# IBM/AdaMML

Measured on AMD Instinct MI355X. Metric: clips/sec (train fwd+bwd) RGB+Audio AdaMML @224^2, 5 seg, higher is better.
Workload: dtype bf16

## Files before the change

adamml_amd/csrc/conv_stem.hip:

```cpp
#include "common.h"
#include "../../include/adamml_hip.h"


namespace {

constexpr int NT = 256;
constexpr int KSTEPS = 7;
constexpr int KTOT = KSTEPS * 32;
constexpr int WROW = KTOT * 2 + 16;
constexpr int MAXPX = 256;
constexpr int SROW = 128 + 8;
constexpr int MAXSLOT = 6;

struct StemP {
    const bf16_t* x;
    const bf16_t* w;
    bf16_t* y;
    double* stats;
    int N, H, W, xc, OH, OW;
    int R;
    int tiles_per_img, total_tiles, tpb;
    int PW, PR;
    size_t gx, gy;
};

__global__ __launch_bounds__(NT, 2) void conv_stem_kernel(StemP p) {
    extern __shared__ __attribute__((aligned(16))) char smem[];
    char* s_w = smem;
    float* cs = reinterpret_cast<float*>(smem + 64 * WROW);
    char* s_patch = smem + 64 * WROW + 512;
    const int tid = threadIdx.x, lane = tid & 63, wave = tid >> 6;
    const int li = lane & 15, lg = lane >> 4;
    const int g = blockIdx.y;
    p.x += (size_t)g * p.gx;
    p.y += (size_t)g * p.gy;

    {
        constexpr int WSL = 64 * (KTOT / 8) / NT;
        static_assert(64 * (KTOT / 8) % NT == 0, "weight slots must divide evenly");
        bf16x8 wv[WSL];
#pragma unroll
        for (int l = 0; l < WSL; ++l) wv[l] = *reinterpret_cast<const bf16x8*>(p.w + (size_t)(tid + l * NT) * 8);
#pragma unroll
        for (int l = 0; l < WSL; ++l) {
            const int e = tid + l * NT;
            const int co = e / (KTOT / 8), ch = e - co * (KTOT / 8);
            *reinterpret_cast<bf16x8*>(s_w + co * WROW + ch * 16) = wv[l];
        }
    }
    if (tid < 128) cs[tid] = 0.f;

    const int pairs_per_row = p.PW >> 1;
    const int nslots = p.PR * pairs_per_row;
    int s_off[MAXSLOT], s_ih[MAXSLOT], s_iw[MAXSLOT];
#pragma unroll
    for (int l = 0; l < MAXSLOT; ++l) {
        const int e = tid + l * NT;
        const int pr = e / pairs_per_row, pc = (e - pr * pairs_per_row) * 2;
        s_ih[l] = e < nslots ? pr : -(1 << 20);
        s_iw[l] = pc - 3;
        s_off[l] = (pr * p.PW + pc) * 8;
    }
    s16x4 ra[MAXSLOT], rb[MAXSLOT];
    unsigned vmask = 0;
    auto load_patch = [&](int tile) {
        const int n = tile / p.tiles_per_img, tr = tile - n * p.tiles_per_img;
        const int ih0 = 2 * tr * p.R - 3;
        vmask = 0;
        const bf16_t* img = p.x + (size_t)n * p.H * p.W * p.xc;
#pragma unroll
        for (int l = 0; l < MAXSLOT; ++l) {
            const int ih = ih0 + s_ih[l], iw = s_iw[l];
            const bool rok = (unsigned)ih < (unsigned)p.H;
            const bf16_t* row = img + (size_t)min(max(ih, 0), p.H - 1) * p.W * p.xc;
            ra[l] = *reinterpret_cast<const s16x4*>(row + min(max(iw, 0), p.W - 1) * p.xc);
            rb[l] = *reinterpret_cast<const s16x4*>(row + min(max(iw + 1, 0), p.W - 1) * p.xc);
            vmask |= ((rok && (unsigned)iw < (unsigned)p.W) ? 1u : 0u) << (2 * l);
            vmask |= ((rok && (unsigned)(iw + 1) < (unsigned)p.W) ? 2u : 0u) << (2 * l);
        }
    };
    const int tile0 = blockIdx.x * p.tpb;
    if (tile0 < p.total_tiles) load_patch(tile0);
    int pixoff[4];
#pragma unroll
    for (int pt = 0; pt < 4; ++pt) {
        int q = (wave * 4 + pt) * 16 + li;
        if (q >= p.R * p.OW) q = 0;
        const int r = q / p.OW, c = q - r * p.OW;
        pixoff[pt] = ((2 * r) * p.PW + 2 * c + 2 * lg) * 8;
    }

    for (int it = 0; it < p.tpb; ++it) {
        const int tile = tile0 + it;
        if (tile >= p.total_tiles) break;
        const int n = tile / p.tiles_per_img, tr = tile - n * p.tiles_per_img;
        const int oh0 = tr * p.R;
        const int rows = min(p.R, p.OH - oh0);
        const int npx = rows * p.OW;
#pragma unroll
        for (int l = 0; l < MAXSLOT; ++l) {
            if (tid + l * NT < nslots) {
                union { struct { s16x4 a, b; } s; bf16x8 v; } u;
                u.s.a = (vmask >> (2 * l)) & 1u ? ra[l] : s16x4{0, 0, 0, 0};
                u.s.b = (vmask >> (2 * l)) & 2u ? rb[l] : s16x4{0, 0, 0, 0};
                *reinterpret_cast<bf16x8*>(s_patch + s_off[l]) = u.v;
            }
        }
        __syncthreads();
        if (it + 1 < p.tpb && tile + 1 < p.total_tiles) load_patch(tile + 1);

        f32x4 acc[4][4];
#pragma unroll
        for (int pt = 0; pt < 4; ++pt)
#pragma unroll
            for (int ct = 0; ct < 4; ++ct) acc[ct][pt] = f32x4{0.f, 0.f, 0.f, 0.f};
        const int rowbytes = p.PW * 8;
#pragma unroll
        for (int kh = 0; kh < KSTEPS; ++kh) {
            bf16x8 fw[4];
#pragma unroll
            for (int ct = 0; ct < 4; ++ct) fw[ct] = *reinterpret_cast<const bf16x8*>(s_w + (ct * 16 + li) * WROW + kh * 64 + lg * 16);
            bf16x8 fa[4];
#pragma unroll
            for (int pt = 0; pt < 4; ++pt) fa[pt] = *reinterpret_cast<const bf16x8*>(s_patch + pixoff[pt] + kh * rowbytes);
#pragma unroll
            for (int pt = 0; pt < 4; ++pt)
#pragma unroll
                for (int ct = 0; ct < 4; ++ct)
                    acc[ct][pt] = __builtin_amdgcn_mfma_f32_16x16x32_bf16(fw[ct], fa[pt], acc[ct][pt], 0, 0, 0);
        }
        __syncthreads();

#pragma unroll
        for (int pt = 0; pt < 4; ++pt) {
            const int q = (wave * 4 + pt) * 16 + li;
#pragma unroll
            for (int ct = 0; ct < 4; ++ct) {
                bf16x4 v = f32_to_bf4(acc[ct][pt]);
                if (q >= npx) v = bf16x4{0, 0, 0, 0};
                *reinterpret_cast<bf16x4*>(s_patch + q * SROW + (ct * 16 + lg * 4) * 2) = v;
            }
        }
        __syncthreads();
        bf16_t* ybase = p.y + ((size_t)n * p.OH + oh0) * p.OW * 64;
        for (int e = tid; e < npx * 8; e += NT) {
            const int q = e >> 3, ch = e & 7;
            const s16x4 lo = *reinterpret_cast<const s16x4*>(s_patch + q * SROW + ch * 16);
            const s16x4 hi = *reinterpret_cast<const s16x4*>(s_patch + q * SROW + ch * 16 + 8);
            union { struct { s16x4 a, b; } s; bf16x8 v; } u;
            u.s.a = lo; u.s.b = hi;
            *reinterpret_cast<bf16x8*>(ybase + (size_t)q * 64 + ch * 8) = u.v;
        }
        if (p.stats) {
            union { s16x4 h[2]; bf16x8 v; } ones;
            ones.h[0] = s16x4{0x3F80, 0x3F80, 0x3F80, 0x3F80};
            ones.h[1] = ones.h[0];
            const int trow = 8 * lg + (li >> 2);
            f32x4 dsum = {0.f, 0.f, 0.f, 0.f}, dsq = {0.f, 0.f, 0.f, 0.f};
            const int nps = (npx + 31) >> 5;
            for (int ps = 0; ps < nps; ++ps) {
                const char* fp = s_patch + (ps * 32 + trow) * SROW + (wave * 16 + 4 * (li & 3)) * 2;
                union { s16x4 h[2]; bf16x8 v; } f;
                f.h[0] = __builtin_amdgcn_ds_read_tr16_b64_v4i16((__attribute__((address_space(3))) s16x4*)(fp));
                f.h[1] = __builtin_amdgcn_ds_read_tr16_b64_v4i16((__attribute__((address_space(3))) s16x4*)(fp + 4 * SROW));
                dsum = __builtin_amdgcn_mfma_f32_16x16x32_bf16(ones.v, f.v, dsum, 0, 0, 0);
                dsq = __builtin_amdgcn_mfma_f32_16x16x32_bf16(f.v, f.v, dsq, 0, 0, 0);
            }
            if (lg == 0) cs[wave * 16 + li] += dsum[0];
            if ((li >> 2) == lg) {
                const int r = li & 3;
                cs[64 + wave * 16 + li] += r == 0 ? dsq[0] : r == 1 ? dsq[1] : r == 2 ? dsq[2] : dsq[3];
            }
        }
        __syncthreads();
    }
    if (p.stats) {
        __syncthreads();
        if (tid < 128) det_add(p.stats + (size_t)g * ADAMML_STAT_SLOTS * 128 + tid, 128, cs[tid]);
    }
}

struct StemWP {
    const bf16_t* x;
    const bf16_t* dz;
    float* ws;
    int N, H, W, xc, OH, OW, R, tiles_per_img, total_tiles, tpb, PW, PR;
};

constexpr int DZROW = 128 + 8;
constexpr int MAXDZ = 8;

__global__ __launch_bounds__(NT, 2) void conv_stem_wgrad_kernel(StemWP p) {
    extern __shared__ __attribute__((aligned(16))) char smem[];
    char* s_patch = smem;
    char* s_dz = smem + ((p.PR * p.PW * 8 + 15) & ~15);
    const int tid = threadIdx.x, lane = tid & 63, wave = tid >> 6;
    const int li = lane & 15, lg = lane >> 4;
    const int pairs_per_row = p.PW >> 1;
    const int nslots = p.PR * pairs_per_row;
    int s_off[MAXSLOT], s_ih[MAXSLOT], s_iw[MAXSLOT];
#pragma unroll
    for (int l = 0; l < MAXSLOT; ++l) {
        const int e = tid + l * NT;
        const int pr = e / pairs_per_row, pc = (e - pr * pairs_per_row) * 2;
        s_ih[l] = e < nslots ? pr : -(1 << 20);
        s_iw[l] = pc - 3;
        s_off[l] = (pr * p.PW + pc) * 8;
    }
    s16x4 ra[MAXSLOT], rb[MAXSLOT];
    bf16x8 rz[MAXDZ];
    unsigned vmask = 0;
    auto load_tile = [&](int tile) {
        const int n = tile / p.tiles_per_img, tr = tile - n * p.tiles_per_img;
// ... 128 lines not shown
    }
}

__global__ void pack_stem_weight_kernel(const float* w, bf16_t* out, int cin_true) {
    const int e = blockIdx.x * blockDim.x + threadIdx.x;
    if (e >= 64 * KTOT) return;
    const int c = e & 3, kw = (e >> 2) & 7, kh = (e >> 5) % 7, co = e / KTOT;
    float v = 0.f;
    if (kw < 7 && c < cin_true) v = w[((size_t)(co * cin_true + c) * 7 + kh) * 7 + kw];
    reinterpret_cast<__bf16*>(out)[e] = (__bf16)v;
}

}

extern "C" int adamml_pack_stem_weight(const float* w, void* out, int cout, int cin_true, hipStream_t stream) {
    if (!w || !out) return adamml_set_error(ADAMML_EINVAL, "pack_stem_weight: null argument");
    if (cout != 64 || cin_true < 1 || cin_true > 4)
        return adamml_set_error(ADAMML_EUNSUPPORTED, "pack_stem_weight: needs cout == 64 and 1..4 input channels (cout=%d cin=%d)", cout, cin_true);
    hipLaunchKernelGGL(pack_stem_weight_kernel, dim3(ceil_div(64 * KTOT, 256)), dim3(256), 0, stream, w, (bf16_t*)out, cin_true);
    return adamml_check_launch("pack_stem_weight");
}

extern "C" int adamml_conv_stem_supported(const adamml_conv_desc_t* d) {
    if (!d) return 0;
    if (d->KH != 7 || d->KW != 7 || d->stride != 2 || d->pad != 3 || d->Cout != 64 || (d->Cin != 8 && d->Cin != 4)) return 0;
    if (d->W % 2 || d->OW != d->W / 2 || d->OH != (d->H + 6 - 7) / 2 + 1 || d->OW > MAXPX || d->OW < 1) return 0;
    const int R = MAXPX / d->OW;
    const int PR = 2 * R + 5, PW = d->W + 6;
    const size_t patch = (size_t)PR * PW * 8, stage = (size_t)MAXPX * SROW;
    if (PR * (PW / 2) > MAXSLOT * NT) return 0;
    return 64 * WROW + 512 + (patch > stage ? patch : stage) <= 64 * 1024;
}

extern "C" int adamml_conv_stem_fwd(const adamml_conv_desc_t* d, const void* x, const void* w_stem_packed, void* y, double* stats,
                                    hipStream_t stream) {
    if (!d || !x || !w_stem_packed || !y) return adamml_set_error(ADAMML_EINVAL, "conv_stem_fwd: null argument");
    if (!adamml_conv_stem_supported(d))
        return adamml_set_error(ADAMML_EUNSUPPORTED, "conv_stem_fwd: needs a 7x7/2 pad 3 conv of a <=4-channel (8-padded) image to 64 "
                                "channels with even W <= %d*2 (H=%d W=%d Cin=%d Cout=%d)", MAXPX, d->H, d->W, d->Cin, d->Cout);
    StemP p;
    p.x = (const bf16_t*)x; p.w = (const bf16_t*)w_stem_packed; p.y = (bf16_t*)y; p.stats = stats;
    p.N = d->N; p.H = d->H; p.W = d->W; p.xc = d->Cin; p.OH = d->OH; p.OW = d->OW;
    p.R = MAXPX / d->OW;
    if (p.R > d->OH) p.R = d->OH;
    p.PR = 2 * p.R + 5; p.PW = d->W + 6;
    p.tiles_per_img = ceil_div(d->OH, p.R);
    p.total_tiles = d->N * p.tiles_per_img;
    if (p.total_tiles <= 0) return ADAMML_OK;
    const int groups = d->groups < 1 ? 1 : d->groups;
    p.gx = (size_t)d->N * d->H * d->W * d->Cin;
    p.gy = (size_t)d->N * d->OH * d->OW * 64;
    p.tpb = (int)(((long)p.total_tiles * groups + 1535) / 1536);
    if (p.tpb < 1) p.tpb = 1;
    const size_t patch = (size_t)p.PR * p.PW * 8, stage = (size_t)MAXPX * SROW;
    const size_t lds = 64 * WROW + 512 + (patch > stage ? patch : stage);
    hipLaunchKernelGGL(conv_stem_kernel, dim3(ceil_div(p.total_tiles, p.tpb), groups), dim3(NT), lds, stream, p);
    return adamml_check_launch("conv_stem_fwd");
}

static int stem_wgrad_blocks(const adamml_conv_desc_t* d, int* tpb_out) {
    const int R = MAXPX / d->OW > d->OH ? d->OH : MAXPX / d->OW;
    const long total = (long)(d->groups < 1 ? 1 : d->groups) * d->N * ceil_div(d->OH, R);
    int tpb = (int)((total + 767) / 768);
    if (tpb < 1) tpb = 1;
    *tpb_out = tpb;
    return (int)((total + tpb - 1) / tpb);
}

extern "C" size_t adamml_conv_stem_bwd_weight_workspace(const adamml_conv_desc_t* d) {
    if (!d || !adamml_conv_stem_supported(d)) return 0;
    int tpb;
    return (size_t)stem_wgrad_blocks(d, &tpb) * 64 * KTOT * sizeof(float);
}

extern "C" int adamml_conv_stem_bwd_weight(const adamml_conv_desc_t* d, const void* dz, const void* x, float* dw, int cin_true,
                                           void* workspace, size_t workspace_bytes, hipStream_t stream) {
    if (!d || !dz || !x || !dw || !workspace) return adamml_set_error(ADAMML_EINVAL, "conv_stem_bwd_weight: null argument");
    if (!adamml_conv_stem_supported(d) || cin_true < 1 || cin_true > 4)
        return adamml_set_error(ADAMML_EUNSUPPORTED, "conv_stem_bwd_weight: not a stem shape (see adamml_conv_stem_supported)");
    StemWP p;
    p.x = (const bf16_t*)x; p.dz = (const bf16_t*)dz; p.ws = (float*)workspace;
    p.N = d->N * (d->groups < 1 ? 1 : d->groups);
    p.H = d->H; p.W = d->W; p.xc = d->Cin; p.OH = d->OH; p.OW = d->OW;
    p.R = MAXPX / d->OW;
    if (p.R > d->OH) p.R = d->OH;
    p.PR = 2 * p.R + 5; p.PW = d->W + 6;
    p.tiles_per_img = ceil_div(d->OH, p.R);
    p.total_tiles = p.N * p.tiles_per_img;
    if (p.total_tiles <= 0) return ADAMML_OK;
    const int nblk = stem_wgrad_blocks(d, &p.tpb);
// ... 12 lines not shown
```

adamml_amd/hip.py:

```python
import ctypes
import os
from ctypes import c_void_p, c_int, c_int32, c_int64, c_float, c_double, c_size_t, c_char_p, POINTER, Structure, byref

import torch

_HERE = os.path.dirname(os.path.abspath(__file__))
LIB_PATH = os.environ.get("ADAMML_HIP_LIB") or os.path.join(_HERE, "libadamml_hip.so")

ACT_NONE, ACT_RELU, ACT_RELU6 = 0, 1, 2
STAT_SLOTS = 32


class ConvDesc(Structure):
    _fields_ = [(n, c_int32) for n in ("N", "H", "W", "Cin", "OH", "OW", "Cout", "KH", "KW", "stride", "pad", "up", "act",
                                      "accumulate", "groups", "in_gstride")]

    def __init__(self, *args, **kw):
        super().__init__(*args, **kw)
        if self.groups < 1:
            self.groups = 1


_P, _I, _F, _D, _Z, _L = c_void_p, c_int, c_float, c_double, c_size_t, c_int64
_DESC = POINTER(ConvDesc)

SIGNATURES = {
    "adamml_conv_fwd": [_DESC, _P, _P, _P, _P, _P, _P, _P],
    "adamml_conv_bwd_data": [_DESC, _P, _P, _P, _I, _P],
    "adamml_conv_fwd_bn_add": [_DESC, _P, _P, _P, _P, _P, _P, _P, _P, _I, _I, _P, _P, _P],
    "adamml_conv_fwd_bn_add_next": [_DESC, _P, _P, _P, _P, _P, _P, _P, _P, _I, _I, _P, _P, _P, _P, _P, _P],
    "adamml_conv_fwd_bn_add_tpool": [_DESC, _P, _P, _P, _P, _P, _P, _P, _P, _I, _I, _I, _P, _P, _P],
    "adamml_temporal_pool_bwd_code": [_P, _P, _P, _P, _I, _I, _I, _I, _I, _P],
    "adamml_temporal_pool_bwd_code_prod": [_P, _P, _P, _P, _P, _P, _P, _I, _I, _P, _P, _Z, _I, _I, _I, _I, _I, _I, _P],
    "adamml_copy2d": [_P, _Z, _P, _Z, _Z, _Z, _P],
    "adamml_gram_stats": [_P, _P, _P, _P, _I, _I, _I, _P],
    "adamml_gram_colsum": [_P, _P, _P, _I, _I, _P, _P, _Z, _I, _I, _P, _Z, _P],
    "adamml_conv_bwd_data_bn": [_DESC, _P, _P, _P, _P, _P, _I, _P, _P],
    "adamml_bn_bwd_affine": [_P, _P, _P, _I, _I, _P],
    "adamml_conv_bwd_data_dual": [_DESC, _P, _P, _P, _P, _P, _P, _I, _P, _P, _I, _P, _P],
    "adamml_conv_bwd_weight_grouped": [_DESC, _P, _P, _P, _I, _I, _P, _P, _P, _P, _I, _P, _Z, _P],
    "adamml_lazy_colsum": [_P, _P, _P, _I, _I, _P, _Z, _I, _I, _P],
    "adamml_alg_sumfix": [_P, _P, _P, _P, _I, _I, _I, _P],
    "adamml_alg_pack": [_P, _P, _P, _P, _P, _I, _I, _I, _P],
    "adamml_alg_wgrad_combine": [_P, _P, _P, _P, _P, _P, _P, _I, _I, _I, _P],
    "adamml_conv_bwd_data_alg": [_DESC, _P, _P, _P, _P, _P, _P, _P, _I, _P, _P, _I, _P, _P],
    "adamml_conv_bwd_data_res": [_DESC, _P, _P, _P, _I, _P, _P, _I, _P, _P, _P, _P, _P, _P, _P],
    "adamml_conv_bwd_data_res_prod": [_DESC, _P, _P, _P, _P, _I, _P, _P, _P, _P, _I, _I, _I, _P, _P, _Z, _P],
    "adamml_bn_act_add_mask": [_P, _P, _P, _I, _I, _P, _P, _P, _I, _P, _P, _Z, _I, _I, _P],
# ... 98 lines not shown
    lib.adamml_conv_bwd_data_alg_streams.restype = c_int
    lib.adamml_conv_fused_input_supported.argtypes = [_DESC]
    lib.adamml_conv_fused_input_supported.restype = c_int
    lib.adamml_conv1x1_narrow_supported.argtypes = [_DESC, c_int]
    lib.adamml_conv1x1_narrow_supported.restype = c_int
    lib.adamml_conv1x1_wide_supported.argtypes = [_DESC, c_int]
    lib.adamml_conv1x1_wide_supported.restype = c_int
    lib.adamml_conv_fwd_bn_add_supported.argtypes = [_DESC]
    lib.adamml_conv_fwd_bn_add_supported.restype = c_int
    lib.adamml_conv_fwd_bn_add_next_supported.argtypes = [_DESC, c_int]
    lib.adamml_conv_fwd_bn_add_next_supported.restype = c_int
    lib.adamml_conv_fwd_bn_add_tpool_supported.argtypes = [_DESC, _I, _I, _I]
    lib.adamml_conv_fwd_bn_add_tpool_supported.restype = c_int
    lib.adamml_conv_bwd_data_dual_supported.argtypes = [_DESC]
    lib.adamml_conv_bwd_data_dual_supported.restype = c_int
    lib.adamml_conv_bwd_data_res_supported.argtypes = [_DESC]
    lib.adamml_conv_bwd_data_res_supported.restype = c_int
    lib.adamml_temporal_pool_bwd_res_supported.argtypes = [_I, _I, _I]
    lib.adamml_temporal_pool_bwd_res_supported.restype = c_int
    lib.adamml_dwconv_bwd_data_bn_supported.argtypes = [_DESC]
    lib.adamml_dwconv_bwd_data_bn_supported.restype = c_int
    lib.adamml_temporal_pool_bwd_code_prod_supported.argtypes = [c_int, c_int, c_int]
    lib.adamml_temporal_pool_bwd_code_prod_supported.restype = c_int
    lib.adamml_temporal_pool_bwd_code_prod_workspace.argtypes = [c_int, c_int, c_int, c_int, c_int, c_int]
    lib.adamml_temporal_pool_bwd_code_prod_workspace.restype = c_size_t
    lib.adamml_dwconv_bwd_fused_supported.argtypes = [_DESC]
    lib.adamml_dwconv_bwd_fused_supported.restype = c_int
    lib.adamml_dwconv_bwd_fused_workspace.argtypes = [_DESC]
    lib.adamml_dwconv_bwd_fused_workspace.restype = c_size_t
    lib.adamml_jpeg_decode_workspace.argtypes = [_L]
    lib.adamml_jpeg_decode_workspace.restype = c_size_t
    lib.adamml_conv_stem_supported.argtypes = [_DESC]
    lib.adamml_conv_stem_supported.restype = c_int
    lib.adamml_plan_run.argtypes = [c_void_p, c_int, c_void_p, c_int, c_void_p, c_int, c_void_p, c_int]
    lib.adamml_plan_run.restype = c_int
    lib.adamml_plan_events_create.argtypes = [c_void_p, c_int]
    lib.adamml_plan_events_create.restype = c_int
    lib.adamml_plan_events_destroy.argtypes = [c_void_p, c_int]
    lib.adamml_plan_events_destroy.restype = c_int
    lib.adamml_plan_num_entry_points.restype = c_int
    lib.adamml_pack_block_elems.restype = c_int
    lib.adamml_version.restype = c_int
    lib.adamml_last_error_string.restype = c_char_p
    lib.adamml_set_deterministic.argtypes = [_I]
    lib.adamml_set_deterministic.restype = c_int
    lib.adamml_get_deterministic.restype = c_int
    _lib = lib
    return lib


def set_deterministic(on=True):
    lib = _lib if _lib is not None else load()
    rc = lib.adamml_set_deterministic(1 if on else 0)
    if rc != 0:
        raise RuntimeError("adamml_set_deterministic failed (%d): %s" % (rc, lib.adamml_last_error_string().decode()))


def deterministic():
    return bool((_lib if _lib is not None else load()).adamml_get_deterministic())


_raw_stream = getattr(torch._C, "_cuda_getCurrentRawStream", None)


def _stream():
    if _raw_stream is not None:
# ... 101 lines not shown
```

adamml_amd/resnet.py:

```python
import torch
import torch.nn as nn

from . import hip
from .backbone import HipBackbone, FlatBuffers, StockDDPAware
from .common import MeanStdMixin
from .runtime import (Lazy, conv_bn, conv_bn_add, conv_bn_add_supported, conv_bn_add_tpool_supported, add_act, maxpool3x3s2, temporal_pool, head, clip_to_nhwc, pad8,
                      ACT_NONE, ACT_RELU)

__all__ = ['ResNet', 'resnet']

_BLOCKS = {50: [3, 4, 6, 3], 101: [3, 4, 23, 3], 152: [3, 8, 36, 3]}


class _Bottleneck(nn.Module):
    expansion = 4

    def __init__(self, inplanes, planes, stride, downsample):
        super().__init__()
        self.conv1 = nn.Conv2d(inplanes, planes, 1, bias=False)
        self.bn1 = nn.BatchNorm2d(planes)
        self.conv2 = nn.Conv2d(planes, planes, 3, stride, 1, bias=False)
        self.bn2 = nn.BatchNorm2d(planes)
        self.conv3 = nn.Conv2d(planes, planes * 4, 1, bias=False)
        self.bn3 = nn.BatchNorm2d(planes * 4)
        self.downsample = downsample
        self.stride = stride


class ResNet(HipBackbone, MeanStdMixin, StockDDPAware):

    def __init__(self, depth, num_frames, num_classes=1000, dropout=0.5, zero_init_residual=False,
                 without_t_stride=False, pooling_method='max', input_channels=3):
        super().__init__()
        self._install_ddp_probe()
        if depth not in _BLOCKS:
            raise ValueError("adamml_amd.ResNet: the HIP path implements the Bottleneck depths 50/101/152 "
                             "(the AdaMML hot path uses 50); got depth=%r" % (depth,))
        layers = _BLOCKS[depth]
        self.pooling_method = pooling_method.lower()
# ... 13 lines not shown
        self.layer4 = self._make_layer(512, layers[3], stride=2)
        self.dropout_p = dropout
        self.fc = nn.Linear(2048, num_classes)

        self._stem = self._register_conv(self.conv1)
        for layer in (self.layer1, self.layer2, self.layer3, self.layer4):
            for b in layer:
                b._cs1 = self._register_conv(b.conv1)
                b._cs2 = self._register_conv(b.conv2)
                b._cs3 = self._register_conv(b.conv3)
                b._csd = self._register_conv(b.downsample[0]) if b.downsample is not None else None
        self.flat_owner = FlatBuffers(self)

    def _make_layer(self, planes, blocks, stride=1):
        downsample = None
        if stride != 1 or self.inplanes != planes * 4:
            downsample = nn.Sequential(nn.Conv2d(self.inplanes, planes * 4, 1, stride, bias=False),
                                       nn.BatchNorm2d(planes * 4))
        layers = [_Bottleneck(self.inplanes, planes, stride, downsample)]
        self.inplanes = planes * 4
        for _ in range(1, blocks):
            layers.append(_Bottleneck(self.inplanes, planes, 1, None))
        return nn.Sequential(*layers)

    def _run(self, x, groups, need_grad):
        rt = self.rt
        tape = rt.begin_forward(x.device, self.training, need_grad, groups)
        self._repack(need_grad)
        frames = self.orig_num_frames
        nt = x.shape[0]
        n = nt // frames
        h = Lazy(x, requires_grad=False)
        self._mark_grads_ready_after(tape, [self.conv1, self.bn1, self.layer1, self.layer2])
        h = conv_bn(rt, h, self._stem, self.bn1, ACT_RELU)
        h = maxpool3x3s2(rt, h, sole_consumer=True)
        for li, layer in enumerate((self.layer1, self.layer2, self.layer3, self.layer4)):
            if li == 2:
                self._mark_grads_ready_after(tape, [self.layer3])
            elif li == 3:
                self._mark_grads_ready_after(tape, [self.layer4, self.fc])
            for bi, b in enumerate(layer):
                idn = conv_bn(rt, h, b._csd, b.downsample[1], ACT_NONE) if b._csd is not None else h
                o = conv_bn(rt, h, b._cs1, b.bn1, ACT_RELU, last_consumer=b._csd is None)
                o = conv_bn(rt, o, b._cs2, b.bn2, ACT_RELU, sole_consumer=True)
                pooled = False
                if conv_bn_add_supported(rt, o, b._cs3, need_grad, idn):
                    pooled = (b is layer[-1] and li < 3 and not self.without_t_stride and
                              conv_bn_add_tpool_supported(rt, o, b._cs3, idn, ACT_RELU, frames, self.pooling_method))
                    nxt = layer[bi + 1]._cs1 if (bi + 1 < len(layer) and not pooled) else None
                    h = conv_bn_add(rt, o, b._cs3, b.bn3, idn, ACT_RELU, idn_sole=b._csd is not None, tpool=frames if pooled else 0, next_cs=nxt)
                else:
                    o = conv_bn(rt, o, b._cs3, b.bn3, ACT_NONE, sole_consumer=True)
                    h = add_act(rt, o, idn, ACT_RELU, idn_sole=b._csd is not None)
            if li < 3 and not self.without_t_stride:
                if not pooled:
                    h = temporal_pool(rt, h, frames, self.pooling_method, sole_consumer=True)
                frames = max(1, frames // 2)
        out, head_backward = head(rt, h, self.fc, frames, self.dropout_p if self.training else 0.0, getattr(self, "_dropout_keep_mask", None))
        rt.end_forward()
        if need_grad:
            tape.record(lambda: head_backward(tape.grad_out))
        return out, tape

    def forward(self, x):
        hip.require_gpu(x)
        self.flat_owner.ensure(x.device)
        if self.training and torch.is_grad_enabled():
            self.flat_owner.ensure_grads()
# ... 28 lines not shown
```

adamml_amd/runtime.py:

```python
import collections
import math
import torch
import torch.distributed as dist

from . import hip, interleave
from .hip import ConvDesc, ACT_NONE, ACT_RELU, ACT_RELU6, STAT_SLOTS, call, ptr
from ctypes import byref

BN_EPS = 1e-5
BN_MOMENTUM = 0.1

R_1X1 = "conv1x1_streaming"
R_FUSED = "conv1x1_fused_streaming"
R_KXK = "convKxK_mfma"
R_WGRAD = "weight_gradient"


def pad8(c):
    return (c + 7) // 8 * 8


class Lazy:
    __slots__ = ("data", "scale", "shift", "gs", "act", "grad", "requires_grad", "vec", "src", "pre_sums", "res", "res_done", "pool_grad", "alg", "sums_partial",
                 "recompute", "_shape", "alg_in", "prod", "next_pre")
# ... 73 lines not shown
        self.off += n
        self.high = max(self.high, self.off)
        return t


class SyncCtx:

    def __init__(self, group=None, enabled=False, force=False):
        self.group = group
        ok = enabled and dist.is_available() and dist.is_initialized()
        self.world = dist.get_world_size(group) if ok else 1
        self.enabled = bool(ok and (self.world > 1 or force))

    def reduce(self, t, C, groups):
        if not self.enabled:
            return t, STAT_SLOTS
        return interleave.exchange_stats(t, C, groups, self.group), 1


class NetRT:

    def __init__(self):
        self.fwd_arena = Arena()
        self.bwd_arena = Arena()
        self.sync = SyncCtx()
        self.training = False
        self.groups = 1
        self.tape = Tape(False)
        self.wgrad_stream = None
        self.wgrad_pending = collections.deque()
        self.capture = None
        self.pre_pending = 0
        self.pre_dropped = 0
        self.state_gen = 0

    def begin_forward(self, device, training, need_grad, groups=1):
        self.training = training
        self.groups = groups
        self.tape = Tape(need_grad)
        self.touched_bns = []
        self.pre_pending = 0
        if training:
            self.fwd_arena.reset(device)
        return self.tape

    def end_forward(self):
        self.pre_dropped += self.pre_pending
        self.pre_pending = 0
        if self.training and self.touched_bns:
            torch._foreach_add_([b.num_batches_tracked for b in self.touched_bns], self.groups)
            self.state_gen += 1
            if hip.recorder is not None:
                nbt, grp = [b.num_batches_tracked for b in self.touched_bns], self.groups

                def bump():
                    torch._foreach_add_(nbt, grp)
                    self.state_gen += 1
                hip.recorder.post_fwd.append(bump)
        self.touched_bns = []


class ConvState:

    def __init__(self, weight, stride, pad, depthwise=False):
        self.weight = weight
        self.cout, self.cin_true, self.kh, self.kw = weight.shape
# ... 732 lines not shown
        self.shape, self.device = shape, device


def maxpool3x3s2(rt, x, sole_consumer=False):
    n, h, w, C = x.shape
    oh, ow = (h + 2 - 3) // 2 + 1, (w + 2 - 3) // 2 + 1
    y = torch.empty(n, oh, ow, C, dtype=torch.bfloat16, device=x.data.device)
    idx = torch.empty(n, oh, ow, C, dtype=torch.uint8, device=x.data.device)
    G = rt.groups
    fuse_bn = sole_consumer and rt.tape.need_grad and x.requires_grad and x.vec is not None
    zsel = torch.empty_like(y) if fuse_bn else None
    call("adamml_maxpool2d_fwd", ptr(x.data), ptr(x.scale), ptr(x.shift), x.gs, x.act, ptr(y), ptr(idx), ptr(zsel), n // G, h, w, C, oh, ow, G)
    out = Lazy(y)
    if rt.capture is not None and "aux" in rt.capture:
        rt.capture["aux"][id(out)] = idx
    if rt.tape.need_grad:
        def bwd():
            g = out.grad
            out.grad = None
            if g is None or not x.requires_grad:
                return
            if sole_consumer and x.grad is None and x.vec is not None and x.pre_sums is None:
                x.pool_grad = (g, idx, zsel, oh, ow)
                return
            acc = 1
            if x.grad is None:
                x.grad = torch.empty_like(x.data)
                acc = 0
            call("adamml_maxpool2d_bwd", ptr(g), ptr(idx), ptr(x.grad), n, h, w, C, oh, ow, acc)
        rt.tape.record(bwd)
    return out


def temporal_pool(rt, x, frames, mode, sole_consumer=False):
    nt, h, w, C = x.shape
    G = rt.groups
    nb = nt // frames
    to = (frames - 1) // 2 + 1
    m = {"max": 0, "avg": 1}.get(mode)
    if m is None:
        raise ValueError("only support avg or max")
    y = torch.empty(nb * to, h, w, C, dtype=torch.bfloat16, device=x.data.device)
    call("adamml_temporal_pool_fwd", ptr(x.data), ptr(x.scale), ptr(x.shift), x.gs, x.act, ptr(y), nb // G, frames, h * w * C, C, m, G)
    out = Lazy(y)
    if rt.tape.need_grad:
        def bwd():
            g = out.grad
            out.grad = None
            if g is None or not x.requires_grad:
                return
            gx = torch.empty_like(x.data)
            if sole_consumer and x.grad is None and x.scale is None and x.res is not None and not x.res_done and \
                    hip.load().adamml_temporal_pool_bwd_res_supported(frames, C, m):
                z, idn, ract, idn_sole, _ = x.res
                fb = idn is not None and idn_sole and idn.requires_grad and idn.vec is not None and idn.grad is None
                if z.requires_grad and z.vec is not None and z.grad is None and z.pre_sums is None and not fb:
                    sa = rt.bwd_arena.take(G * 2 * C * STAT_SLOTS)
                    call("adamml_temporal_pool_bwd_res", ptr(g), ptr(x.data), ract, ptr(gx), None if z.alg else ptr(z.data), ptr(z.vec), ptr(sa),
                         nb // G, frames, h * w, C, G)
                    z.pre_sums = sa
                    z.sums_partial = z.alg
                    x.res_done = True
                    x.grad = gx
                    return
            call("adamml_temporal_pool_bwd", ptr(g), ptr(x.data), ptr(x.scale), ptr(x.shift), x.gs, x.act, ptr(gx), nb // G, frames,
                 h * w * C, C, m, G)
# ... 196 lines not shown
```

include/adamml_hip.h:

```cpp
#ifndef ADAMML_HIP_H
#define ADAMML_HIP_H
#include <stddef.h>
#include <stdint.h>
#ifdef __cplusplus
extern "C" {
#endif

typedef struct ihipStream_t* hipStream_t;
typedef struct ihipEvent_t* hipEvent_t;

#define ADAMML_API __attribute__((visibility("default")))

#define ADAMML_STAT_SLOTS 32

#define ADAMML_ACT_NONE 0
#define ADAMML_ACT_RELU 1
#define ADAMML_ACT_RELU6 2

typedef struct {
    int32_t N, H, W, Cin;
    int32_t OH, OW, Cout;
    int32_t KH, KW, stride, pad;
    int32_t up;
    int32_t act;
    int32_t accumulate;
    int32_t groups;
    int32_t in_gstride;
} adamml_conv_desc_t;

ADAMML_API int adamml_version(void);
ADAMML_API const char* adamml_last_error_string(void);
ADAMML_API int adamml_set_deterministic(int on);
ADAMML_API int adamml_get_deterministic(void);

ADAMML_API int adamml_conv_fwd(const adamml_conv_desc_t* d, const void* x, const void* w_packed, const float* in_scale,
                    const float* in_shift, void* y, double* stats, hipStream_t stream);
ADAMML_API int adamml_conv_fused_input_supported(const adamml_conv_desc_t* d);
ADAMML_API int adamml_conv1x1_narrow_supported(const adamml_conv_desc_t* d, int kind);
ADAMML_API int adamml_conv1x1_wide_supported(const adamml_conv_desc_t* d, int kind);
ADAMML_API int adamml_conv_fwd_bn_add_supported(const adamml_conv_desc_t* d);
ADAMML_API int adamml_conv_fwd_bn_add_streams(const adamml_conv_desc_t* d);
ADAMML_API int adamml_conv_fwd_bn_add(const adamml_conv_desc_t* d, const void* x, const void* w_packed, const float* in_scale, const float* in_shift,
                           const float* bn_vec, const void* idn, const float* id_scale, const float* id_shift, int id_gstride, int act,
                           void* out, uint8_t* mask_out, hipStream_t stream);
ADAMML_API int adamml_conv_fwd_bn_add_next_supported(const adamml_conv_desc_t* d, int next_cout);
ADAMML_API int adamml_conv_fwd_bn_add_next(const adamml_conv_desc_t* d, const void* x, const void* w_packed, const float* in_scale, const float* in_shift,
                                const float* bn_vec, const void* idn, const float* id_scale, const float* id_shift, int id_gstride, int act,
                                void* out, uint8_t* mask_out, const void* w_next, void* y_next, double* stats_next, hipStream_t stream);
ADAMML_API int adamml_conv_fwd_bn_add_tpool_supported(const adamml_conv_desc_t* d, int frames, int act, int lazy_input);
ADAMML_API int adamml_conv_fwd_bn_add_tpool_streams(const adamml_conv_desc_t* d, int frames);
ADAMML_API int adamml_conv_fwd_bn_add_tpool(const adamml_conv_desc_t* d, const void* x, const void* w_packed, const float* in_scale, const float* in_shift,
                                 const float* bn_vec, const void* idn, const float* id_scale, const float* id_shift, int id_gstride, int act,
                                 int frames, void* pooled, uint16_t* code, hipStream_t stream);
ADAMML_API int adamml_gram_stats(const void* w_packed, const float* G, const float* s, double* sums, int Cout, int Cin, int groups, hipStream_t stream);
ADAMML_API int adamml_gram_colsum_supported(int C);
ADAMML_API size_t adamml_gram_colsum_workspace(size_t P, int C, int groups);
ADAMML_API int adamml_gram_colsum(const void* x, const float* scale, const float* shift, int gstride, int act, float* G, float* s, size_t P, int C,
                       int groups, void* workspace, size_t workspace_bytes, hipStream_t stream);
ADAMML_API int adamml_conv_bwd_data(const adamml_conv_desc_t* d, const void* dz, const void* w_dgrad_packed, void* dx,
                         int accumulate, hipStream_t stream);
// ... 15 lines not shown
ADAMML_API int adamml_alg_pack(const float* w, const float* aff, const float* m_pre, void* w_alg, float* epi_add, int Cout, int Cin, int groups,
                    hipStream_t stream);
ADAMML_API int adamml_alg_wgrad_combine(const float* w, const float* aff, const float* P, const float* G, const float* wg_pre, const float* s, float* dw,
                             int Cout, int Cin, int groups, hipStream_t stream);
ADAMML_API int adamml_conv_bwd_data_alg_streams(const adamml_conv_desc_t* d);
ADAMML_API int adamml_conv_bwd_data_alg(const adamml_conv_desc_t* d, const void* g, const void* a, const float* a_scale, const float* a_shift,
                             const void* w_alg, const float* epi_add, void* dx, int accumulate, const void* z_in, const float* bn_vec,
                             int act, double* sums, hipStream_t stream);

ADAMML_API int adamml_conv_bwd_data_res_supported(const adamml_conv_desc_t* d);
ADAMML_API int adamml_conv_bwd_data_res_streams(const adamml_conv_desc_t* d);
ADAMML_API int adamml_conv_bwd_data_res(const adamml_conv_desc_t* d, const void* dz, const void* w_dgrad_packed, void* dx,
                             int accumulate, const void* res_out, const uint8_t* res_mask, int res_act, const void* z_a, const float* vec_a,
                             double* sums_a, const void* z_b, const float* vec_b, double* sums_b, hipStream_t stream);

ADAMML_API int adamml_conv_bwd_data_res_prod_supported(const adamml_conv_desc_t* d, int a_channels);
ADAMML_API size_t adamml_conv_bwd_data_res_prod_workspace(const adamml_conv_desc_t* d);
ADAMML_API int adamml_conv_bwd_data_res_prod_streams(const adamml_conv_desc_t* d, int a_channels);
ADAMML_API int adamml_conv_bwd_data_res_prod(const adamml_conv_desc_t* d, const void* dz, const void* w_dgrad_packed, void* dx, const uint8_t* res_mask,
                                  int res_act, double* sums_a, const void* a, const float* a_scale, const float* a_shift, int a_act,
                                  int a_gstride, int a_channels, float* prod, void* workspace, size_t workspace_bytes, hipStream_t stream);

ADAMML_API size_t adamml_conv_bwd_weight_workspace(const adamml_conv_desc_t* d, int cin_true);
ADAMML_API int adamml_conv_bwd_weight(const adamml_conv_desc_t* d, const void* dz, const void* x, const float* in_scale,
                           const float* in_shift, float* dw, int cin_true, void* workspace, size_t workspace_bytes,
                           hipStream_t stream);
ADAMML_API int adamml_pack_conv_weight(const float* w, void* out, int cout, int cin_true, int cin_pad, int kh, int kw, int mode,
                            hipStream_t stream);

ADAMML_API int adamml_conv_stem_supported(const adamml_conv_desc_t* d);
ADAMML_API int adamml_pack_stem_weight(const float* w, void* out, int cout, int cin_true, hipStream_t stream);
ADAMML_API int adamml_conv_stem_fwd(const adamml_conv_desc_t* d, const void* x, const void* w_stem_packed, void* y, double* stats,
                         hipStream_t stream);
ADAMML_API size_t adamml_conv_stem_bwd_weight_workspace(const adamml_conv_desc_t* d);
ADAMML_API int adamml_conv_stem_bwd_weight(const adamml_conv_desc_t* d, const void* dz, const void* x, float* dw, int cin_true,
                                void* workspace, size_t workspace_bytes, hipStream_t stream);

ADAMML_API int adamml_dwconv_fwd(const adamml_conv_desc_t* d, const void* x, const float* w_tapmajor, const float* in_scale,
                      const float* in_shift, void* y, double* stats, hipStream_t stream);
ADAMML_API int adamml_dwconv_bwd_data(const adamml_conv_desc_t* d, const void* dz, const float* w_tapmajor, void* dx,
                           int accumulate, hipStream_t stream);
ADAMML_API int adamml_dwconv_bwd_data_bn_supported(const adamml_conv_desc_t* d);
ADAMML_API int adamml_dwconv_bwd_data_bn(const adamml_conv_desc_t* d, const void* dz, const float* w_tapmajor, void* dx, const void* z_in,
                              const float* bn_vec, int act, double* sums, hipStream_t stream);
ADAMML_API size_t adamml_dwconv_bwd_weight_workspace(const adamml_conv_desc_t* d);
ADAMML_API int adamml_dwconv_bwd_fused_supported(const adamml_conv_desc_t* d);
ADAMML_API size_t adamml_dwconv_bwd_fused_workspace(const adamml_conv_desc_t* d);
ADAMML_API int adamml_dwconv_bwd_fused(const adamml_conv_desc_t* d, const void* g, const void* z, const float* aff, const float* w_tapmajor,
                            const void* x, const float* x_vec, int x_act, void* dx, double* sums, float* dw, void* workspace,
                            size_t workspace_bytes, hipStream_t stream);
ADAMML_API int adamml_conv_stem1_supported(const adamml_conv_desc_t* d);
ADAMML_API int adamml_conv_stem1_fwd(const adamml_conv_desc_t* d, const float* x, size_t image_stride, size_t group_stride, const float* w_tapmajor,
                          void* y, double* stats, hipStream_t stream);
ADAMML_API size_t adamml_conv_stem1_bwd_weight_workspace(const adamml_conv_desc_t* d);
ADAMML_API int adamml_conv_stem1_bwd_weight(const adamml_conv_desc_t* d, const void* dz, const float* x, size_t image_stride, size_t group_stride,
                                 float* dw , void* workspace,
                                 size_t workspace_bytes, hipStream_t stream);
ADAMML_API int adamml_dwconv_bwd_weight(const adamml_conv_desc_t* d, const void* dz, const void* x, const float* in_scale,
                             const float* in_shift, float* dw, void* workspace, size_t workspace_bytes, hipStream_t stream);

ADAMML_API int adamml_stats_collapse(const double* stats, double* out, int C, int groups, hipStream_t stream);
ADAMML_API int adamml_bn_finalize(const double* stats, int nslots, int groups, double count, const float* gamma, const float* beta,
                       float* running_mean, float* running_var, float momentum, float eps, float* bn_vec, int C,
                       hipStream_t stream);
ADAMML_API int adamml_bn_eval_affine(const float* gamma, const float* beta, const float* running_mean, const float* running_var,
                          float eps, float* scale, float* shift, int C, hipStream_t stream);
// ... 124 lines not shown
```

Before: 3484.

## Fuse 3x3/2 maxpool selection into the stem conv kernel using BN gamma sign

```diff
diff --git a/adamml_amd/csrc/conv_stem.hip b/adamml_amd/csrc/conv_stem.hip
--- a/adamml_amd/csrc/conv_stem.hip
+++ b/adamml_amd/csrc/conv_stem.hip
@@ -1,3 +1,4 @@
+#include <limits.h>
 #include "common.h"
 #include "../../include/adamml_hip.h"
 
@@ -11,6 +12,12 @@
 constexpr int MAXPX = 256;
 constexpr int SROW = 128 + 8;
 constexpr int MAXSLOT = 6;
+
+typedef short s16x2 __attribute__((ext_vector_type(2)));
+typedef unsigned short u16x2 __attribute__((ext_vector_type(2)));
+__device__ __forceinline__ unsigned pk_umax(unsigned a, unsigned b) {
+    return __builtin_bit_cast(unsigned, __builtin_elementwise_max(__builtin_bit_cast(u16x2, a), __builtin_bit_cast(u16x2, b)));
+}
 
 struct StemP {
     const bf16_t* x;
@@ -22,18 +29,44 @@
     int tiles_per_img, total_tiles, tpb;
     int PW, PR;
     size_t gx, gy;
+    const float* gamma;
+    bf16_t* z_sel;
+    uint8_t* idx;
+    size_t gz;
 };
 
-__global__ __launch_bounds__(NT, 2) void conv_stem_kernel(StemP p) {
+template <bool POOL>
+__device__ __forceinline__ void conv_stem_body(StemP p) {
     extern __shared__ __attribute__((aligned(16))) char smem[];
     char* s_w = smem;
     float* cs = reinterpret_cast<float*>(smem + 64 * WROW);
-    char* s_patch = smem + 64 * WROW + 512;
+    char* s_patch = smem + 64 * WROW + 512 + (POOL ? p.OW * SROW : 0);
     const int tid = threadIdx.x, lane = tid & 63, wave = tid >> 6;
     const int li = lane & 15, lg = lane >> 4;
     const int g = blockIdx.y;
     p.x += (size_t)g * p.gx;
     p.y += (size_t)g * p.gy;
+    s16x2 sg2[4];
+    int pk_off[2];
+    bool pk_left[2], pk_top[2];
+    if constexpr (POOL) {
+        p.z_sel += (size_t)g * p.gz;
+        if (p.idx) p.idx += (size_t)g * p.gz;
+        const int ch = tid & 7, hw = p.OW >> 1;
+#pragma unroll
+        for (int i = 0; i < 8; ++i) {
+            const float gm = p.gamma[ch * 8 + i];
+            sg2[i >> 1][i & 1] = gm > 0.f ? 1 : gm < 0.f ? -1 : 0;
+        }
+#pragma unroll
+        for (int k = 0; k < 2; ++k) {
+            const int e = (tid + k * NT) >> 3;
+            const int j = e / hw, pw = e - j * hw;
+            pk_off[k] = (2 * j * p.OW + 2 * pw) * SROW + ch * 16;
+            pk_left[k] = pw > 0;
+            pk_top[k] = j > 0;
+        }
+    }
 
     {
         constexpr int WSL = 64 * (KTOT / 8) / NT;
@@ -80,7 +113,8 @@
         }
     };
     const int tile0 = blockIdx.x * p.tpb;
-    if (tile0 < p.total_tiles) load_patch(tile0);
+    const int it0 = (POOL && tile0 < p.total_tiles && tile0 % p.tiles_per_img != 0) ? -1 : 0;
+    if (tile0 < p.total_tiles) load_patch(tile0 + it0);
     int pixoff[4];
 #pragma unroll
     for (int pt = 0; pt < 4; ++pt) {
@@ -90,9 +124,10 @@
         pixoff[pt] = ((2 * r) * p.PW + 2 * c + 2 * lg) * 8;
     }
 
-    for (int it = 0; it < p.tpb; ++it) {
+    for (int it = it0; it < p.tpb; ++it) {
         const int tile = tile0 + it;
         if (tile >= p.total_tiles) break;
+        const bool live = !POOL || it >= 0;
         const int n = tile / p.tiles_per_img, tr = tile - n * p.tiles_per_img;
         const int oh0 = tr * p.R;
         const int rows = min(p.R, p.OH - oh0);
@@ -143,7 +178,7 @@
         }
         __syncthreads();
         bf16_t* ybase = p.y + ((size_t)n * p.OH + oh0) * p.OW * 64;
-        for (int e = tid; e < npx * 8; e += NT) {
+        for (int e = tid; e < (live ? npx * 8 : 0); e += NT) {
             const int q = e >> 3, ch = e & 7;
             const s16x4 lo = *reinterpret_cast<const s16x4*>(s_patch + q * SROW + ch * 16);
             const s16x4 hi = *reinterpret_cast<const s16x4*>(s_patch + q * SROW + ch * 16 + 8);
@@ -151,7 +186,7 @@
             u.s.a = lo; u.s.b = hi;
             *reinterpret_cast<bf16x8*>(ybase + (size_t)q * 64 + ch * 8) = u.v;
         }
-        if (p.stats) {
+        if (p.stats && live) {
             union { s16x4 h[2]; bf16x8 v; } ones;
             ones.h[0] = s16x4{0x3F80, 0x3F80, 0x3F80, 0x3F80};
             ones.h[1] = ones.h[0];
@@ -172,6 +207,91 @@
                 cs[64 + wave * 16 + li] += r == 0 ? dsq[0] : r == 1 ? dsq[1] : r == 2 ? dsq[2] : dsq[3];
             }
         }
+        if constexpr (POOL) {
+            const int nitems = live ? (rows >> 1) * (p.OW >> 1) * 8 : 0;
+            const size_t pbase = (((size_t)n * (p.OH >> 1) + (oh0 >> 1)) * (p.OW >> 1)) * 64;
+            const int rowb = p.OW * SROW;
+#pragma unroll
+            for (int k = 0; k < 2; ++k) {
+                const int e = tid + k * NT;
+                if (e < nitems) {
+                    const char* c0 = s_patch + pk_off[k];
+                    const bool topok = pk_top[k] || tr > 0, leftok = pk_left[k];
+                    int kbest[8];
+                    unsigned det = 0;
+#pragma unroll
+                    for (int i = 0; i < 8; ++i) kbest[i] = INT_MIN;
+#pragma unroll
+                    for (int kh = 0; kh < 3; ++kh)
+#pragma unroll
+                        for (int kw = 0; kw < 3; ++kw) {
+                            const bool ok = (kh > 0 || topok) && (kw > 0 || leftok);
+                            const char* tp = c0 + (kh - 1) * rowb + (kw - 1) * SROW;
+                            const uint2 lo = *reinterpret_cast<const uint2*>(tp), hi = *reinterpret_cast<const uint2*>(tp + 8);
+                            const unsigned w4[4] = {lo.x, lo.y, hi.x, hi.y};
+                            const int tag = 8 - (kh * 3 + kw);
+#pragma unroll
+                            for (int dq = 0; dq < 4; ++dq) {
+                                const unsigned mag = w4[dq] & 0x7FFF7FFFu;
+                                if (kh > 0 && kw > 0) det = pk_umax(det, mag);
+                                else det = pk_umax(det, ok ? mag : 0u);
+                                const s16x2 m = __builtin_bit_cast(s16x2, w4[dq]) >> 15;
+                                const s16x2 kk = ((__builtin_bit_cast(s16x2, mag) ^ m) - m) * sg2[dq];
+                                unsigned ku = __builtin_bit_cast(unsigned, kk);
+                                if (!(kh > 0 && kw > 0)) ku = ok ? ku : 0x80008000u;
+                                kbest[2 * dq] = max(kbest[2 * dq], (int)((ku << 16) | (unsigned)tag));
+                                kbest[2 * dq + 1] = max(kbest[2 * dq + 1], (int)((ku & 0xFFFF0000u) | (unsigned)tag));
+                            }
+                        }
+                    bf16x8 zs;
+                    uint64_t packed = 0;
+                    if ((((det + 0x00800080u) & 0x80008000u) == 0)) {
+#pragma unroll
+                        for (int i = 0; i < 8; ++i) {
+                            const int t = 8 - (kbest[i] & 15);
+                            const int kh = (t * 11) >> 5, kw = t - 3 * kh;
+                            union { uint16_t u; __bf16 h; } r;
+                            r.u = *reinterpret_cast<const uint16_t*>(c0 + (kh - 1) * rowb + (kw - 1) * SROW + 2 * i);
+                            zs[i] = r.h;
+                            packed |= (uint64_t)t << (8 * i);
+                        }
+                    } else {
+                        float best[8];
+                        int bi[8];
+#pragma unroll
+                        for (int i = 0; i < 8; ++i) { best[i] = -INFINITY; bi[i] = 0; zs[i] = 0; }
+#pragma unroll 1
+                        for (int t = 0; t < 9; ++t) {
+                            const int kh = (t * 11) >> 5, kw = t - 3 * kh;
+                            const bool ok = (kh > 0 || topok) && (kw > 0 || leftok);
+                            const char* tp = c0 + (kh - 1) * rowb + (kw - 1) * SROW;
+                            union { struct { s16x4 a, b; } s; bf16x8 v; } u;
+                            u.s.a = *reinterpret_cast<const s16x4*>(tp);
+                            u.s.b = *reinterpret_cast<const s16x4*>(tp + 8);
+                            const f32x8 v = bf8_to_f32(u.v);
+#pragma unroll
+                            for (int i = 0; i < 8; ++i) {
+                                const float key = (float)sg2[i >> 1][i & 1] * v[i];
+                                const bool take = ok && (key > best[i] || __builtin_isnan(key));
+                                best[i] = take ? key : best[i];
+                                bi[i] = take ? t : bi[i];
+                                zs[i] = take ? u.v[i] : zs[i];
+                            }
+                        }
+#pragma unroll
+                        for (int i = 0; i < 8; ++i) packed |= (uint64_t)bi[i] << (8 * i);
+                    }
+                    *reinterpret_cast<bf16x8*>(p.z_sel + pbase + (size_t)e * 8) = zs;
+                    if (p.idx) *reinterpret_cast<uint64_t*>(p.idx + pbase + (size_t)e * 8) = packed;
+                }
+            }
+            __syncthreads();
+            const char* lastrow = s_patch + (rows - 1) * rowb;
+            for (int e = tid; e < p.OW * 16; e += NT) {
+                const int o = (e >> 4) * SROW + (e & 15) * 8;
+                *reinterpret_cast<s16x4*>(s_patch - rowb + o) = *reinterpret_cast<const s16x4*>(lastrow + o);
+            }
+        }
         __syncthreads();
     }
     if (p.stats) {
@@ -179,6 +299,9 @@
         if (tid < 128) det_add(p.stats + (size_t)g * ADAMML_STAT_SLOTS * 128 + tid, 128, cs[tid]);
     }
 }
+
+__global__ __launch_bounds__(NT, 2) void conv_stem_kernel(StemP p) { conv_stem_body<false>(p); }
+__global__ __launch_bounds__(NT, 2) void conv_stem_pool_kernel(StemP p) { conv_stem_body<true>(p); }
 
 struct StemWP {
     const bf16_t* x;
@@ -373,14 +496,19 @@
     return 64 * WROW + 512 + (patch > stage ? patch : stage) <= 64 * 1024;
 }
 
+static int conv_stem_fwd_pool(const adamml_conv_desc_t* d, const void* x, const void* w_stem_packed, const float* gamma, void* y,
+                              double* stats, void* z_sel, uint8_t* idx, hipStream_t stream);
+
 extern "C" int adamml_conv_stem_fwd(const adamml_conv_desc_t* d, const void* x, const void* w_stem_packed, void* y, double* stats,
                                     hipStream_t stream) {
     if (!d || !x || !w_stem_packed || !y) return adamml_set_error(ADAMML_EINVAL, "conv_stem_fwd: null argument");
+    if (d->pool_z_sel) return conv_stem_fwd_pool(d, x, w_stem_packed, d->pool_gamma, y, stats, d->pool_z_sel, d->pool_idx, stream);
     if (!adamml_conv_stem_supported(d))
         return adamml_set_error(ADAMML_EUNSUPPORTED, "conv_stem_fwd: needs a 7x7/2 pad 3 conv of a <=4-channel (8-padded) image to 64 "
                                 "channels with even W <= %d*2 (H=%d W=%d Cin=%d Cout=%d)", MAXPX, d->H, d->W, d->Cin, d->Cout);
     StemP p;
     p.x = (const bf16_t*)x; p.w = (const bf16_t*)w_stem_packed; p.y = (bf16_t*)y; p.stats = stats;
+    p.gamma = nullptr; p.z_sel = nullptr; p.idx = nullptr; p.gz = 0;
     p.N = d->N; p.H = d->H; p.W = d->W; p.xc = d->Cin; p.OH = d->OH; p.OW = d->OW;
     p.R = MAXPX / d->OW;
     if (p.R > d->OH) p.R = d->OH;
@@ -397,6 +525,55 @@
     const size_t lds = 64 * WROW + 512 + (patch > stage ? patch : stage);
     hipLaunchKernelGGL(conv_stem_kernel, dim3(ceil_div(p.total_tiles, p.tpb), groups), dim3(NT), lds, stream, p);
     return adamml_check_launch("conv_stem_fwd");
+}
+
+static size_t stem_pool_lds(const adamml_conv_desc_t* d) {
+    int R = MAXPX / d->OW;
+    if (R > d->OH) R = d->OH;
+    const size_t patch = (size_t)(2 * R + 5) * (d->W + 6) * 8, stage = (size_t)MAXPX * SROW;
+    return 64 * WROW + 512 + (size_t)d->OW * SROW + (patch > stage ? patch : stage);
+}
+
+extern "C" int adamml_conv_stem_pool_supported(const adamml_conv_desc_t* d) {
+    if (!adamml_conv_stem_supported(d)) return 0;
+    int R = MAXPX / d->OW;
+    if (R > d->OH) R = d->OH;
+    if (R % 2 || d->OH % 2 || d->OW % 2) return 0;
+    return 2 * stem_pool_lds(d) <= 160 * 1024;
+}
+
+static int conv_stem_fwd_pool(const adamml_conv_desc_t* d, const void* x, const void* w_stem_packed, const float* gamma, void* y,
+                              double* stats, void* z_sel, uint8_t* idx, hipStream_t stream) {
+    if (!gamma) return adamml_set_error(ADAMML_EINVAL, "conv_stem_fwd (pooled): pool_gamma is null");
+    if (!adamml_conv_stem_pool_supported(d))
+        return adamml_set_error(ADAMML_EUNSUPPORTED, "conv_stem_fwd (pooled): needs a stem shape (adamml_conv_stem_supported) with even OH, OW and "
+                                "rows per strip (H=%d W=%d Cin=%d Cout=%d k=%d)", d->H, d->W, d->Cin, d->Cout, d->KH);
+    StemP p;
+    p.x = (const bf16_t*)x; p.w = (const bf16_t*)w_stem_packed; p.y = (bf16_t*)y; p.stats = stats;
+    p.gamma = gamma; p.z_sel = (bf16_t*)z_sel; p.idx = idx;
+    p.N = d->N; p.H = d->H; p.W = d->W; p.xc = d->Cin; p.OH = d->OH; p.OW = d->OW;
+    p.R = MAXPX / d->OW;
+    if (p.R > d->OH) p.R = d->OH;
+    p.PR = 2 * p.R + 5; p.PW = d->W + 6;
+    p.tiles_per_img = ceil_div(d->OH, p.R);
+    p.total_tiles = d->N * p.tiles_per_img;
+    if (p.total_tiles <= 0) return ADAMML_OK;
+    const int groups = d->groups < 1 ? 1 : d->groups;
+    p.gx = (size_t)d->N * d->H * d->W * d->Cin;
+    p.gy = (size_t)d->N * d->OH * d->OW * 64;
+    p.gz = (size_t)d->N * (d->OH / 2) * (d->OW / 2) * 64;
+    p.tpb = (int)(((long)p.total_tiles * groups + 1535) / 1536);
+    if (p.tpb < 1) p.tpb = 1;
+    const size_t lds = stem_pool_lds(d);
+    static AdamLdsOnce attr_once;
+    const int attr_dev = adamml_current_device();
+    if (!attr_once.test(attr_dev)) {
+        hipError_t e = hipFuncSetAttribute(reinterpret_cast<const void*>(conv_stem_pool_kernel), hipFuncAttributeMaxDynamicSharedMemorySize, (int)lds);
+        if (e != hipSuccess) return adamml_set_error(ADAMML_ELAUNCH, "conv_stem_fwd (pooled): cannot raise the dynamic LDS limit: %s", hipGetErrorString(e));
+        attr_once.set(attr_dev);
+    }
+    hipLaunchKernelGGL(conv_stem_pool_kernel, dim3(ceil_div(p.total_tiles, p.tpb), groups), dim3(NT), lds, stream, p);
+    return adamml_check_launch("conv_stem_fwd (pooled)");
 }
 
 static int stem_wgrad_blocks(const adamml_conv_desc_t* d, int* tpb_out) {
diff --git a/adamml_amd/hip.py b/adamml_amd/hip.py
--- a/adamml_amd/hip.py
+++ b/adamml_amd/hip.py
@@ -13,7 +13,8 @@
 
 class ConvDesc(Structure):
     _fields_ = [(n, c_int32) for n in ("N", "H", "W", "Cin", "OH", "OW", "Cout", "KH", "KW", "stride", "pad", "up", "act",
-                                      "accumulate", "groups", "in_gstride")]
+                                      "accumulate", "groups", "in_gstride")] + \
+               [(n, c_void_p) for n in ("pool_gamma", "pool_z_sel", "pool_idx")]
 
     def __init__(self, *args, **kw):
         super().__init__(*args, **kw)
@@ -178,6 +179,8 @@
     lib.adamml_jpeg_decode_workspace.restype = c_size_t
     lib.adamml_conv_stem_supported.argtypes = [_DESC]
     lib.adamml_conv_stem_supported.restype = c_int
+    lib.adamml_conv_stem_pool_supported.argtypes = [_DESC]
+    lib.adamml_conv_stem_pool_supported.restype = c_int
     lib.adamml_plan_run.argtypes = [c_void_p, c_int, c_void_p, c_int, c_void_p, c_int, c_void_p, c_int]
     lib.adamml_plan_run.restype = c_int
     lib.adamml_plan_events_create.argtypes = [c_void_p, c_int]
diff --git a/adamml_amd/resnet.py b/adamml_amd/resnet.py
--- a/adamml_amd/resnet.py
+++ b/adamml_amd/resnet.py
@@ -4,7 +4,7 @@
 from . import hip
 from .backbone import HipBackbone, FlatBuffers, StockDDPAware
 from .common import MeanStdMixin
-from .runtime import (Lazy, conv_bn, conv_bn_add, conv_bn_add_supported, conv_bn_add_tpool_supported, add_act, maxpool3x3s2, temporal_pool, head, clip_to_nhwc, pad8,
+from .runtime import (Lazy, conv_bn, conv_bn_add, conv_bn_add_supported, conv_bn_add_tpool_supported, add_act, maxpool3x3s2, conv_stem_bn_pool, conv_stem_bn_pool_supported, temporal_pool, head, clip_to_nhwc, pad8,
                       ACT_NONE, ACT_RELU)
 
 __all__ = ['ResNet', 'resnet']
@@ -84,8 +84,11 @@
         n = nt // frames
         h = Lazy(x, requires_grad=False)
         self._mark_grads_ready_after(tape, [self.conv1, self.bn1, self.layer1, self.layer2])
-        h = conv_bn(rt, h, self._stem, self.bn1, ACT_RELU)
-        h = maxpool3x3s2(rt, h, sole_consumer=True)
+        if conv_stem_bn_pool_supported(rt, h, self._stem):
+            h = conv_stem_bn_pool(rt, h, self._stem, self.bn1)
+        else:
+            h = conv_bn(rt, h, self._stem, self.bn1, ACT_RELU)
+            h = maxpool3x3s2(rt, h, sole_consumer=True)
         for li, layer in enumerate((self.layer1, self.layer2, self.layer3, self.layer4)):
             if li == 2:
                 self._mark_grads_ready_after(tape, [self.layer3])
diff --git a/adamml_amd/runtime.py b/adamml_amd/runtime.py
--- a/adamml_amd/runtime.py
+++ b/adamml_amd/runtime.py
@@ -129,6 +129,7 @@
         self.capture = None
         self.pre_pending = 0
         self.pre_dropped = 0
+        self.stem_pool = True
         self.state_gen = 0
 
     def begin_forward(self, device, training, need_grad, groups=1):
@@ -927,6 +928,70 @@
     return out
 
 
+def conv_stem_bn_pool_supported(rt, x, cs):
+    if not (rt.stem_pool and cs.stem and x.scale is None and x.shape[0] % rt.groups == 0):
+        return False
+    if rt.tape.need_grad and not rt.training:
+        return False
+    return bool(hip.load().adamml_conv_stem_pool_supported(byref(cs.desc(x.shape, x.act, rt.groups, x.gs))))
+
+
+def conv_stem_bn_pool(rt, x, cs, bn):
+    G = rt.groups
+    d = cs.desc(x.shape, x.act, G, x.gs)
+    dev = x.data.device
+    C = d.Cout
+    poh, pow_ = d.OH // 2, d.OW // 2
+    count = d.N * d.OH * d.OW
+    need_grad = rt.tape.need_grad
+    y = torch.empty(G * d.N, d.OH, d.OW, C, dtype=torch.bfloat16, device=dev)
+    zsel = torch.empty(G * d.N, poh, pow_, C, dtype=torch.bfloat16, device=dev)
+    idx = torch.empty(G * d.N, poh, pow_, C, dtype=torch.uint8, device=dev) if need_grad else None
+    macs = float(count) * G * C * cs.kh * cs.kw * cs.cin_true
+    in_b, out_b = 2.0 * G * d.N * d.H * d.W * cs.cin_true, 2.0 * G * count * C
+    w_b = 2.0 * C * cs.kh * cs.kw * cs.cin_true
+    pool_b = (3.0 if need_grad else 2.0) * G * d.N * poh * pow_ * C
+    dp = cs.desc(x.shape, x.act, G, x.gs)
+    dp.pool_gamma, dp.pool_z_sel, dp.pool_idx = ptr(bn.weight), ptr(zsel), ptr(idx)
+    hip.next_meta = (2 * macs, in_b + out_b + w_b + pool_b, "conv_stem_kernel", R_KXK)
+    if rt.training:
+        stats = rt.fwd_arena.take(G * 2 * C * STAT_SLOTS)
+        call("adamml_conv_stem_fwd", byref(dp), ptr(x.data), ptr(cs.w_stem), ptr(y), ptr(stats))
+        vec = _bn_vectors(rt, bn, stats, count, C, dev)
+        rt.touched_bns.append(bn)
+        out = Lazy(zsel, vec[0, 0], vec[0, 1], ACT_RELU, gs=4 * C)
+    else:
+        call("adamml_conv_stem_fwd", byref(dp), ptr(x.data), ptr(cs.w_stem), ptr(y), None)
+        vec = _bn_eval_vectors(rt, bn, C, dev)
+        out = Lazy(zsel, vec[0], vec[1], ACT_RELU)
+    if rt.capture is not None:
+        rt.capture.setdefault(id(cs.weight), []).append(y)
+        if "aux" in rt.capture:
+            rt.capture["aux"][id(out)] = idx
+    if need_grad:
+        def bwd():
+            g = out.grad
+            out.grad = None
+            if g is None:
+                return
+            sums = rt.bwd_arena.take(G * 2 * C * STAT_SLOTS)
+            call("adamml_bn_bwd_reduce", ptr(g), ptr(zsel), ptr(vec), ACT_RELU, ptr(sums), d.N * poh * pow_, C, G)
+            sums, nslots = rt.sync.reduce(sums, C, G)
+            coef = torch.empty(G, 3, C, dtype=torch.float32, device=dev)
+            train_bn = bn.weight.requires_grad
+            call("adamml_bn_bwd_finalize", ptr(sums), nslots, G, float(count * rt.sync.world), ptr(bn.weight), ptr(vec),
+                 ptr(bn.weight.grad) if train_bn else None, ptr(bn.bias.grad) if train_bn else None, ptr(coef), C, 1.0 / rt.sync.world)
+            dz = torch.empty_like(y)
+            call("adamml_maxpool2d_bwd_bn_apply", ptr(g), ptr(idx), ptr(y), ptr(vec), ACT_RELU, ptr(coef), ptr(dz), d.N, d.OH, d.OW, C, poh, pow_, G)
+            if cs.weight.requires_grad:
+                with _on_wgrad_stream(rt, (dz, x.data, x.scale)):
+                    hip.next_meta = (2 * macs, in_b + out_b + 2 * w_b, None, R_WGRAD)
+                    ws = hip.wgrad_workspace(d, cs.cin_true, dz.device, stem=True)
+                    call("adamml_conv_stem_bwd_weight", byref(d), ptr(dz), ptr(x.data), ptr(cs.weight.grad), cs.cin_true, ptr(ws), ws.numel() * 4)
+        rt.tape.record(bwd)
+    return out
+
+
 def temporal_pool(rt, x, frames, mode, sole_consumer=False):
     nt, h, w, C = x.shape
     G = rt.groups
diff --git a/include/adamml_hip.h b/include/adamml_hip.h
--- a/include/adamml_hip.h
+++ b/include/adamml_hip.h
@@ -26,6 +26,9 @@
     int32_t accumulate;
     int32_t groups;
     int32_t in_gstride;
+    const float* pool_gamma;
+    void* pool_z_sel;
+    uint8_t* pool_idx;
 } adamml_conv_desc_t;
 
 ADAMML_API int adamml_version(void);
@@ -107,6 +110,7 @@
 ADAMML_API int adamml_pack_stem_weight(const float* w, void* out, int cout, int cin_true, hipStream_t stream);
 ADAMML_API int adamml_conv_stem_fwd(const adamml_conv_desc_t* d, const void* x, const void* w_stem_packed, void* y, double* stats,
                          hipStream_t stream);
+ADAMML_API int adamml_conv_stem_pool_supported(const adamml_conv_desc_t* d);
 ADAMML_API size_t adamml_conv_stem_bwd_weight_workspace(const adamml_conv_desc_t* d);
 ADAMML_API int adamml_conv_stem_bwd_weight(const adamml_conv_desc_t* d, const void* dz, const void* x, float* dw, int cin_true,
                                 void* workspace, size_t workspace_bytes, hipStream_t stream);
```

Measured after the change: 3496 (median of 6 runs). About the same (+0.3%).
